# PreferredAI/cornac

Measured on AMD Instinct MI355X. Metric: bpr_triplets_per_sec, higher is better.
Workload: dtype f32

## Files before the change

cornac_amd/csrc/bpr.hip:

```cpp
#include <algorithm>
#include <numeric>
#include <queue>

#include "common.h"
#include "rng.h"
#include "sgd_device.h"

namespace chip {

__global__ __launch_bounds__(kBlock) void bpr_det_sample_kernel(
    const uint32_t *__restrict__ pos_draw, int pos_stride, const uint32_t *__restrict__ neg_draw, int neg_stride,
    int64_t n, const int32_t *__restrict__ user_ids, const int32_t *__restrict__ indices,
    const int32_t *__restrict__ indptr, int neg_population, int32_t *__restrict__ su, int32_t *__restrict__ si,
    int32_t *__restrict__ sj, unsigned long long *__restrict__ counters) {
    const int64_t s = (int64_t)blockIdx.x * kBlock + threadIdx.x;
    bool skip = false;
    if (s < n) {
        const uint32_t ii = pos_draw[s * pos_stride];
        const uint32_t jj = neg_draw[s * neg_stride];
        const int32_t u = user_ids[ii];
        const int32_t i = indices[ii];
        const int32_t j = neg_population == CORNAC_HIP_NEG_POPULARITY ? indices[jj] : (int32_t)jj;
        skip = csr_row_contains(indices, indptr[u], indptr[u + 1], j);
        su[s] = skip ? -1 : u;
// ... 1474 lines not shown
    const int grid = di.cus * h->strata_blocks_per_cu;
    const int64_t W = (int64_t)grid * kWavesPerBlock;
    if (h->own_waves != W) h->strata_built = false;
    build_ownership(h, W);
    build_item_ranks(h);
    h->rec_u.ensure((size_t)h->nnz);
    h->rec_i.ensure((size_t)h->nnz);
    h->sptr.ensure((size_t)W * 8 + 1);
    REQUIRE(grid % 8 == 0, "the strata grid must be a multiple of the 8 XCDs");
    h->strata_claim.ensure(8 * 16);
    return grid;
}

static void strata_build_buckets(cornac_hip_bpr_t h, int grid, uint32_t key) {
    if (h->strata_built && h->strata_key_built == key) return;
    StrataArgs s;
    s.own_u = h->own_u.p; s.own_i = h->own_i.p; s.wave_ptr = h->wave_ptr.p; s.item_rank = h->item_rank.p;
    s.rec_u = h->rec_u.p; s.rec_i = h->rec_i.p; s.sptr = h->sptr.p;
    s.key = key; s.n_hot = h->strata_n_hot; s.n_waves = (int64_t)grid * kWavesPerBlock;
    h->strata_own_code.ensure((size_t)h->nnz);
    s.own_code = h->strata_own_code.p;
    if (h->strata_code_waves != h->own_waves) {
        hipLaunchKernelGGL(strata_code_kernel, dim3((unsigned)std::min<int64_t>(4096, (h->nnz + kBlock - 1) / kBlock)),
                           dim3(kBlock), 0, h->stream, s, h->nnz);
        h->strata_code_waves = h->own_waves;
    }
    hipLaunchKernelGGL(strata_bucket_kernel, dim3(grid), dim3(kBlock), 0, h->stream, s);
    HIP_CHECK(hipGetLastError());
    h->strata_built = true;
    h->strata_key_built = key;
    ++h->strata_builds;
}

static void strata_enqueue(cornac_hip_bpr_t h, int64_t n_samples, float lr, float reg, int use_bias, int flags) {
    const int grid = strata_prepare(h);
    const bool packed = h->strata_allow_pack && ((h->V.owned && h->B.owned) || h->chunk_records) &&
                        !prof_env_set("CORNAC_HIP_STRATA_NO_PACK");
    if (packed) strata_pack(h); else strata_unpack(h);
    if (!packed) h->Bpad.ensure((size_t)h->total_items * kBiasStride);
    const unsigned bgrid = (unsigned)((h->total_items + kBlock - 1) / kBlock);
    int64_t left = n_samples;
    while (left > 0) {
        const int64_t n = std::min(left, h->nnz - h->hog_offset);
        const auto first_phase = [&](int64_t s) { return (int)((8 * (__int128)s + h->nnz - 1) / h->nnz); };
        const int p_lo = first_phase(h->hog_offset), p_hi = h->hog_offset + n >= h->nnz ? 8 : first_phase(h->hog_offset + n);
        if (p_hi > p_lo) {
            uint32_t key = strata_key(h->hog_seed, h->hog_epoch / (uint32_t)std::max(1, h->strata_rehash_period));
            if (prof_env_int("CORNAC_HIP_STRATA_CONTIG", 0)) key = 0x12345u;
            strata_build_buckets(h, grid, key);
            HogArgs a;
            fill_hog_args(h, a, h->nnz, lr, reg, use_bias, CORNAC_HIP_NEG_UNIFORM, flags);
            const bool dense_bias = !packed && prof_env_int("CORNAC_HIP_STRATA_DENSE_BIAS", 0) != 0;
            a.B = dense_bias ? h->B.p : h->Bpad.p;
            a.bstride = dense_bias ? 1 : kBiasStride;
            if (packed) {
                a.V = h->VB.p;
                a.vpitch = h->vb_pitch;
                a.B = h->VB.p + h->vb_kp;
                a.bstride = h->vb_pitch;
            }
            a.rec_u = h->rec_u.p; a.rec_i = h->rec_i.p; a.rank_item = h->rank_item.p; a.sptr = h->sptr.p;
            a.strata_key = key; a.n_hot = h->strata_n_hot;
            HIP_CHECK(hipMemsetAsync(h->strata_claim.p, 0, 8 * 16 * sizeof(uint32_t), h->stream));
            if (!dense_bias && !packed)
                hipLaunchKernelGGL(bias_pad_kernel, dim3(bgrid), dim3(kBlock), 0, h->stream, h->B.p, h->Bpad.p, h->total_items);
            for (int ph = p_lo; ph < p_hi; ++ph) {
                a.phase = ph;
                a.xcd_claim = h->strata_claim.p + 16 * ph;
                h->ktimer.before(h->stream);
                hipLaunchKernelGGL(h->strata_kernel, dim3(grid), dim3(kBlock), 0, h->stream, a);
                h->ktimer.after(h->stream);
            }
            if (!dense_bias && !packed)
                hipLaunchKernelGGL(bias_unpad_kernel, dim3(bgrid), dim3(kBlock), 0, h->stream, h->Bpad.p, h->B.p, h->total_items);
            HIP_CHECK(hipGetLastError());
        }
        advance_hog_offset(h, n);
        left -= n;
    }
}

typedef void (*LdsBinKernel)(const LdsBinArgs);
constexpr int kLdsbinPresampleDefault = 0;
static LdsBinKernel pick_ldsbin_kernel(int k, bool pop, bool exch = false, bool passing = false, bool conv = false, bool pre = false) {
    if (pre) {
        if (k <= 64) return bpr_ldsbin_kernel<1, 4, false, false, 1, false, true>;
        return bpr_ldsbin_kernel<2, 2, false, false, 1, false, true>;
    }
    if (conv) {
        if (pop) {
            if (k <= 64) return bpr_ldsbin_kernel<1, 4, true, false, 1, true>;
            if (k <= 128) return bpr_ldsbin_kernel<2, 4, true, false, 1, true>;
            if (k <= 192) return bpr_ldsbin_kernel<3, 2, true, false, 1, true>;
            return bpr_ldsbin_kernel<4, 1, true, false, 1, true>;
        }
        if (k <= 64) return bpr_ldsbin_kernel<1, 4, false, false, 1, true>;
        if (k <= 128) return bpr_ldsbin_kernel<2, 4, false, false, 1, true>;
        if (k <= 192) return bpr_ldsbin_kernel<3, 2, false, false, 1, true>;
        return bpr_ldsbin_kernel<4, 1, false, false, 1, true>;
    }
    if (passing && !exch && k > 64 && k <= 128) {
#ifdef CORNAC_PROFILE
        if (prof_env_int("CORNAC_HIP_LDSBIN_UNR", 0) == 0)
#endif
            return pop ? bpr_ldsbin_kernel<2, 4, true> : bpr_ldsbin_kernel<2, 4>;
    }
    if (exch) {
        if (pop) {
            if (k <= 64) return bpr_ldsbin_kernel<1, 4, true, true>;
            if (k <= 128) return bpr_ldsbin_kernel<2, 2, true, true>;
            if (k <= 192) return bpr_ldsbin_kernel<3, 2, true, true>;
            return bpr_ldsbin_kernel<4, 1, true, true>;
        }
        if (k <= 64) return bpr_ldsbin_kernel<1, 4, false, true>;
        if (k <= 128) return bpr_ldsbin_kernel<2, 2, false, true>;
        if (k <= 192) return bpr_ldsbin_kernel<3, 2, false, true>;
        return bpr_ldsbin_kernel<4, 1, false, true>;
    }
    if (pop) {
        if (k <= 64) return bpr_ldsbin_kernel<1, 4, true>;
        if (k <= 128) return bpr_ldsbin_kernel<2, 2, true>;
        if (k <= 192) return bpr_ldsbin_kernel<3, 2, true>;
        return bpr_ldsbin_kernel<4, 1, true>;
    }
#ifdef CORNAC_PROFILE
    if (k <= 64) switch (prof_env_int("CORNAC_HIP_LDSBIN_UNR", 0)) {
        case 1: return bpr_ldsbin_kernel<1, 1>;
        case 2: return bpr_ldsbin_kernel<1, 2>;
        case 8: return bpr_ldsbin_kernel<1, 8>;
        default: break;
    }
    else if (k <= 128) switch (prof_env_int("CORNAC_HIP_LDSBIN_UNR", 0)) {
        case 3: return bpr_ldsbin_kernel<2, 3>;
        case 4: return bpr_ldsbin_kernel<2, 4>;
        case 22: return bpr_ldsbin_kernel<2, 2, false, false, 2>;
        case 32: return bpr_ldsbin_kernel<2, 3, false, false, 2>;
        case 42: return bpr_ldsbin_kernel<2, 4, false, false, 2>;
        default: break;
    }
#endif
    if (k <= 64) return bpr_ldsbin_kernel<1, 4>;
    if (k <= 128) return bpr_ldsbin_kernel<2, 2>;
    if (k <= 192) return bpr_ldsbin_kernel<3, 2>;
    return bpr_ldsbin_kernel<4, 1>;
}

constexpr size_t kLbLdsBudget = 96 * 1024;
constexpr size_t kLbLdsExclusive = 82 * 1024;
static size_t ldsbin_lds_bytes(int cap, int k, int waves = kLbWaves) {
    const int kp = ((k + kWave - 1) / kWave) * kWave;
    return ((size_t)cap * (kp + 5) + 1) * sizeof(float) + (size_t)waves * 3 * kWave * sizeof(int32_t);
}

struct LbPlan {
    int bins = 0, block = kLbBlock, cap = 0;
    size_t lds = 0;
    bool passing = false;
};
static LbPlan ldsbin_plan(cornac_hip_bpr_t h) {
    LbPlan pl;
    const int cus = device_info(h->device).cus;
    if (h->cv_blocks) {
        if (h->k > 256) return pl;
        const int waves = h->lb_pass_waves;
        const size_t budget = (size_t)h->lb_pass_kb << 10;
        const int kp = ((h->k + kWave - 1) / kWave) * kWave;
        const size_t fixed = sizeof(float) + (size_t)waves * 3 * kWave * sizeof(int32_t);
        if (budget <= fixed) return pl;
        const int64_t cap_lds = (int64_t)((budget - fixed) / ((size_t)(kp + 5) * sizeof(float)));
        const int64_t cap_min = std::max<int64_t>(h->lb_min_candidates, 16);
        if (cap_lds < cap_min) return pl;
        int64_t bins = (h->n_items + cap_lds - 1) / cap_lds;
        const int64_t more = std::min<int64_t>(h->n_items / (cap_min + cap_min / 3), (int64_t)2 * cus * h->cv_blocks);
        bins = std::max(bins, more);
        bins = std::max<int64_t>(1, (bins + h->cv_blocks - 1) / h->cv_blocks) * h->cv_blocks;
        const int64_t cap = (h->n_items + bins - 1) / bins;
        if (cap > cap_lds || bins > (int64_t(1) << 22) || bins * cap >= (int64_t(1) << 31)) return pl;
        pl.bins = (int)bins;
        pl.cap = (int)cap;
        pl.block = waves * kWave;
        pl.lds = ldsbin_lds_bytes((int)cap, h->k, waves);
        pl.passing = true;
        return pl;
    }
    if (h->k > 256 || h->nnz < (int64_t)cus * kLbWaves * kWave) return pl;
    const int res_waves = prof_env_int("CORNAC_HIP_LDSBIN_RES_WAVES", kLbWaves);
    for (int rounds = prof_env_int("CORNAC_HIP_LDSBIN_MIN_ROUNDS", 1); rounds <= h->lb_max_rounds; ++rounds) {
        const int64_t bins = (int64_t)cus * rounds;
        const int64_t cap = (h->n_items + bins - 1) / bins;
        if (cap < h->lb_min_candidates) return pl;
        if (ldsbin_lds_bytes((int)cap, h->k, res_waves) <= (size_t)prof_env_int("CORNAC_HIP_LDSBIN_BUDGET_KB", (int)(kLbLdsBudget >> 10)) << 10) {
            pl.bins = (int)bins;
            pl.cap = (int)cap;
            pl.block = res_waves * kWave;
            pl.lds = std::max(ldsbin_lds_bytes((int)cap, h->k, res_waves), (size_t)prof_env_int("CORNAC_HIP_LDSBIN_EXCL_KB", (int)(kLbLdsExclusive >> 10)) << 10);
            return pl;
        }
    }
    if (!h->lb_pass_enable || (double)h->nnz * 100.0 < (double)h->n_items * h->lb_pass_min_draws_x100) return pl;
    const int waves = prof_env_int("CORNAC_HIP_LDSBIN_PASS_WAVES", h->lb_pass_waves);
    const size_t budget = (size_t)prof_env_int("CORNAC_HIP_LDSBIN_PASS_KB", h->lb_pass_kb) << 10;
    const int kp = ((h->k + kWave - 1) / kWave) * kWave;
    const size_t fixed = sizeof(float) + (size_t)waves * 3 * kWave * sizeof(int32_t);
    if (budget <= fixed) return pl;
    int64_t cap = (int64_t)((budget - fixed) / ((size_t)(kp + 5) * sizeof(float)));
    if (cap < h->lb_min_candidates) return pl;
    int64_t bins = (h->n_items + cap - 1) / cap;
    bins = ((bins + cus - 1) / cus) * cus;
    cap = (h->n_items + bins - 1) / bins;
    if (cap < h->lb_min_candidates || bins > (int64_t(1) << 22)) return pl;
    pl.bins = (int)bins;
    pl.cap = (int)cap;
    pl.block = waves * kWave;
    pl.lds = ldsbin_lds_bytes((int)cap, h->k, waves);
    pl.passing = true;
    return pl;
}

static bool ldsbin_can_run(cornac_hip_bpr_t h, int64_t n_samples, int neg_population) {
    if (neg_population == CORNAC_HIP_NEG_POPULARITY && h->neg_pop_n) return false;
    const LbPlan pl = ldsbin_plan(h);
    return pl.bins > 0 && (!pl.passing || n_samples * 4 >= h->nnz);
}

static void ldsbin_build(cornac_hip_bpr_t h) {
    const LbPlan plan = ldsbin_plan(h);
    const int bins = plan.bins;
// ... 768 lines not shown
```

cornac_amd/csrc/bpr_ldsbin.inc:

```


namespace chip {

constexpr int kLbBlock = 1024;
constexpr int kLbWaves = kLbBlock / kWave;
constexpr int32_t kLbHot = (int32_t)0x80000000;
constexpr int kLbMaxExchanges = 32;
constexpr int kLbMaxRanges = 8;

struct LdsBinExchange {
    float *base;
    float *bucket;
    float *keep;
    unsigned int *arrive;
    const unsigned int *landed;
    unsigned int *applied;
    long long bucket_stride, keep_stride;
    long long nt;
    int n_ex, rule;
};

struct LdsBinArgs {
    const int32_t *cptr, *cusers;
    const int32_t *rank_item;
    const int32_t *hot_u, *hot_i;
    const uint32_t *hot_off;
    const int32_t *indptr, *indices;
    const uint32_t *bitmap;
    float *U, *V, *B;
    unsigned long long *counters;
    uint64_t seed;
    uint32_t epoch, key;
    int32_t n_items, n_bins, n_hot, n_hot_inter, bm_words, cap;
    int32_t n_strata;
    unsigned long long *wg_clock;
    int k, use_bias;
    float lr, reg;
    int ablate;
    int neg_pop;
    uint64_t s_begin, n, nnz;
    LdsBinExchange ex;
    int32_t conv_bpb;
    int32_t conv_first[kLbMaxRanges];
    float *conv_rows[kLbMaxRanges];
    int32_t *pre_rec;
    uint32_t *pre_cnt;
    const uint32_t *pre_base;
    uint32_t pre_waves;
};

__host__ __device__ __forceinline__ uint32_t ldsbin_rot(uint32_t g, uint32_t key, uint32_t n_bins) {
    uint32_t h = g * 0x9E3779B1u + key;
    h ^= h >> 15; h *= 0x85EBCA77u;
    h ^= h >> 13; h *= 0xC2B2AE3Du;
    h ^= h >> 16;
    return h % n_bins;
}

__host__ __device__ __forceinline__ uint32_t ldsbin_mix(uint32_t h) { return mix32(h); }
__host__ __device__ __forceinline__ uint32_t ldsbin_perm(uint32_t x, uint32_t n, uint32_t key) { return feistel_perm(x, n, key); }

__host__ __device__ inline uint32_t ldsbin_deal_rank(uint32_t p, uint32_t key, uint32_t n_bins, uint32_t n_items,
                                                     uint32_t n_groups, uint32_t n_strata) {
    const uint32_t g = p / n_bins;
    uint32_t s = (uint32_t)(((uint64_t)g * n_strata) / n_groups);
    if ((uint32_t)(((uint64_t)(s + 1u) * n_groups) / n_strata) <= g) ++s;
    const uint32_t g_lo = (uint32_t)(((uint64_t)s * n_groups) / n_strata);
    const uint32_t g_hi = (uint32_t)(((uint64_t)(s + 1u) * n_groups) / n_strata);
    const uint32_t base = g_lo * n_bins;
    const uint64_t end = (uint64_t)g_hi * n_bins;
    const uint32_t size = (uint32_t)(end < (uint64_t)n_items ? end : (uint64_t)n_items) - base;
    return base + ldsbin_perm(p - base, size, key ^ ldsbin_mix(s * 0x27D4EB2Fu + 0x165667B1u));
}

#ifdef CORNAC_PROFILE
#define LB_ABLATE(bit) ((a.ablate & (bit)) != 0)
#else
#define LB_ABLATE(bit) false
#endif

__host__ __device__ __forceinline__ float ex_rule_factor(int rule, float w_sum, float s_norm2) {
    if (rule == 0) return 1.f / sqrtf(fmaxf(w_sum, 1.f));
    return s_norm2 > 0.f ? fminf(1.f, w_sum / s_norm2) : 1.f;
}
__device__ __forceinline__ void store_f32_system(float *p, float v) {
// ... 233 lines not shown
        uint32_t run = 0;
        for (uint32_t g0 = 0; g0 < n_groups; g0 += kWave) {
            const uint32_t g = g0 + lane;
            uint32_t v = g < n_groups ? cum[g + 1] : 0u;
#pragma unroll
            for (int o = 1; o < kWave; o <<= 1) {
                const uint32_t t = __shfl_up(v, o, kWave);
                if (lane >= o) v += t;
            }
            if (g < n_groups) cum[g + 1] = run + v;
            run += __shfl(v, kWave - 1, kWave);
        }
        if (lane == 0) {
            cum[0] = 0;
            *sh_next_tile = 0;
            *sh_cold_mass = run;
            *sh_nslots = (n_groups && item[n_groups - 1] == -1) ? n_groups - 1 : n_groups;
        }
    }
    __syncthreads();
}

template <bool POP>
__device__ __forceinline__ LdsBinDraw ldsbin_draw(const LdsBinArgs &a, const LdsBinCtx &c, uint32_t local, bool in_range) {
    LdsBinDraw d;
    d.in_range = in_range;
    uint32_t w[4];
    philox4x32_10(d.in_range ? local : 0u, c.b, a.epoch, 0x20u, (uint32_t)a.seed, (uint32_t)(a.seed >> 32), w);
    const uint32_t r_pos = lemire_bounded2(w[0], w[1], c.n_draws, c.th_draw);
    uint32_t s_j, excl = 0, excl_lo = 0xffffffffu;
    if (r_pos < c.cold_mass) {
        uint32_t lo = 0, hi = c.n_slots;
        while (hi - lo > 1) {
            const uint32_t mid = (lo + hi) >> 1;
            if (c.cum[mid] <= r_pos) lo = mid; else hi = mid;
        }
        d.u = a.cusers[c.cp[lo] + (int32_t)(r_pos - c.cum[lo])];
        d.ei = (int32_t)lo;
        s_j = c.n_slots > 1 ? lemire_bounded2(w[2], w[3], c.n_slots - 1, c.th_slot1) : 0u;
        if (c.n_slots > 1 && s_j >= lo) ++s_j;
        excl_lo = c.cum[lo];
        excl = c.cum[lo + 1] - excl_lo;
    } else {
        const uint32_t h = c.hot_lo + (r_pos - c.cold_mass);
        d.u = a.hot_u[h];
        d.ei = a.hot_i[h] | kLbHot;
        s_j = lemire_bounded2(w[2], w[3], c.n_slots, c.th_slot);
    }
    if (POP) {
        const uint32_t m = c.n_draws - excl;
        uint32_t r_neg = (uint32_t)(((uint64_t)w[2] * m) >> 32);
        if (r_neg >= excl_lo) r_neg += excl;
        if (m == 0) {
            d.j = c.item[d.ei] & ~kLbHot;
            d.ej = d.ei;
        } else if (r_neg < c.cold_mass) {
            uint32_t lo = 0, hi = c.n_slots;
            while (hi - lo > 1) {
                const uint32_t mid = (lo + hi) >> 1;
                if (c.cum[mid] <= r_neg) lo = mid; else hi = mid;
            }
            d.j = c.item[lo];
            d.ej = (int32_t)lo;
        } else {
            d.j = a.hot_i[c.hot_lo + (r_neg - c.cold_mass)];
            d.ej = d.j | kLbHot;
        }
        return d;
    }
    const int32_t itj = c.item[s_j];
    d.j = itj & ~kLbHot;
    d.ej = itj < 0 ? itj : (int32_t)s_j;
    return d;
}

__device__ __forceinline__ void ldsbin_launch_range(const LdsBinArgs &a, uint32_t n_draws, uint32_t n_waves, uint32_t &d_lo,
                                                    uint32_t &d_hi, uint32_t &tile_w, uint32_t &n_tiles) {
    d_lo = (uint32_t)(((unsigned __int128)n_draws * a.s_begin) / a.nnz);
    d_hi = a.s_begin + a.n >= a.nnz ? n_draws : (uint32_t)(((unsigned __int128)n_draws * (a.s_begin + a.n)) / a.nnz);
    tile_w = (d_hi - d_lo) < 8u * n_waves * kWave ? 32u : 64u;
    n_tiles = (d_hi - d_lo + tile_w - 1) / tile_w;
}

template <int R, int UNR, bool POP = false, bool EXCH = false, int PF = 1, bool CONV = false, bool PRE = false>
__global__ __launch_bounds__(kLbBlock) void bpr_ldsbin_kernel(const LdsBinArgs a) {
    constexpr int G = kWave, KP = G * R, NREF = 2 * UNR;
    extern __shared__ float lb_smem[];
    float *const rows = lb_smem;
    float *const bias = rows + (size_t)a.cap * KP;
    int32_t *const item = reinterpret_cast<int32_t *>(bias + a.cap);
    int32_t *const cp = item + a.cap;
    uint32_t *const cum = reinterpret_cast<uint32_t *>(cp + a.cap);
    int *const lock = reinterpret_cast<int *>(cum + a.cap + 1);
    int32_t(*const stage)[3][kWave] = reinterpret_cast<int32_t(*)[3][kWave]>(lock + a.cap);
    const int wave = threadIdx.x >> 6, lane = lane_id();
    const uint32_t n_waves = blockDim.x >> 6;
    uint32_t b = blockIdx.x;
    const uint32_t nb = (uint32_t)a.n_bins;
    float *cvV = nullptr, *cvB = nullptr;
    if (CONV) {
        const uint32_t r = blockIdx.x / (uint32_t)a.conv_bpb, o = blockIdx.x - r * (uint32_t)a.conv_bpb;
        b = (uint32_t)a.conv_first[r] + o;
        cvV = a.conv_rows[r] + (size_t)o * (size_t)a.cap * (size_t)a.k;
        cvB = a.conv_rows[r] + (size_t)a.conv_bpb * (size_t)a.cap * (size_t)a.k + (size_t)o * (size_t)a.cap;
    }
    const uint32_t n_groups = ((uint32_t)a.n_items + nb - 1) / nb;
#ifdef CORNAC_PROFILE
    if (a.wg_clock && threadIdx.x == 0) a.wg_clock[2 * b] = wall_clock64();
#endif
    __shared__ uint32_t sh_nslots, sh_cold_mass, sh_next_tile;
    __shared__ uint32_t sh_ex_done[kLbMaxExchanges], sh_ex_applied[kLbWaves];
    __shared__ int sh_ex_lock[kLbWaves];
    if (EXCH) {
        if (threadIdx.x < kLbMaxExchanges) sh_ex_done[threadIdx.x] = 0;
        if (threadIdx.x < kLbWaves) {
            sh_ex_applied[threadIdx.x] = 0;
            sh_ex_lock[threadIdx.x] = 0;
        }
    }
    ldsbin_build_tables(a, b, nb, n_groups, item, cp, cum, lock, &sh_nslots, &sh_cold_mass, &sh_next_tile);
    const uint32_t n_slots = sh_nslots, cold_mass = sh_cold_mass;
    const uint32_t hot_lo = a.hot_off[b], hot_share = a.hot_off[b + 1] - hot_lo;
    const uint32_t n_draws = n_slots ? cold_mass + hot_share : 0u;
    const uint32_t th_draw = n_draws ? lemire_thresh(n_draws) : 0u, th_slot = n_slots ? lemire_thresh(n_slots) : 0u,
                   th_slot1 = n_slots > 1 ? lemire_thresh(n_slots - 1) : 0u;
    bool inb[R];
#pragma unroll
    for (int r = 0; r < R; ++r) inb[r] = lane + G * r < a.k;
    {
        constexpr int NL = R <= 2 ? 4 : 2;
        for (uint32_t s0 = wave; s0 < n_slots; s0 += n_waves * NL) {
            float t[NL][R], tb[NL];
            int32_t its[NL];
#pragma unroll
            for (int q = 0; q < NL; ++q) {
                const uint32_t sq = s0 + (uint32_t)q * n_waves;
                its[q] = sq < n_slots ? item[sq] : -1;
                const size_t it = (size_t)(its[q] >= 0 ? its[q] : 0);
                const float *pv = CONV ? cvV + (size_t)(its[q] >= 0 ? sq : 0u) * a.k : a.V + it * a.k;
                const float *pb = CONV ? cvB + (its[q] >= 0 ? sq : 0u) : a.B + it;
#pragma unroll
                for (int r = 0; r < R; ++r) t[q][r] = (its[q] >= 0 && inb[r]) ? pv[lane + G * r] : 0.f;
                tb[q] = (its[q] >= 0 && lane == 0) ? *pb : 0.f;
            }
#pragma unroll
            for (int q = 0; q < NL; ++q) {
                if (its[q] < 0) continue;
                const uint32_t sq = s0 + (uint32_t)q * n_waves;
#pragma unroll
                for (int r = 0; r < R; ++r) rows[(size_t)sq * KP + lane + G * r] = t[q][r];
                if (lane == 0) bias[sq] = tb[q];
            }
        }
    }
    __syncthreads();
    unsigned int n_correct = 0, n_skipped = 0;
    if (!PRE && n_slots == 0 && wave == 0 && lane == 0 && a.s_begin == 0) n_skipped = cold_mass + hot_share;
    uint32_t d_lo, d_hi, tile_w, n_tiles;
    ldsbin_launch_range(a, n_draws, n_waves, d_lo, d_hi, tile_w, n_tiles);
    const LdsBinCtx ctx{item, cp, cum, b, n_slots, cold_mass, hot_lo, n_draws, th_draw, th_slot, th_slot1};
    typedef LdsBinDraw Draws;
    auto draw_tile = [&](uint32_t tile) {
        const uint32_t local = d_lo + tile * tile_w + lane;
        return ldsbin_draw<POP>(a, ctx, local, tile < n_tiles && (uint32_t)lane < tile_w && local < d_hi);
    };
    auto member_word = [&](const Draws &d) -> uint32_t {
        return (a.bitmap && !LB_ABLATE(1)) ? a.bitmap[(size_t)d.u * a.bm_words + (d.j >> 5)] : 0u;
    };
    auto member_bounds = [&](const Draws &d, int32_t &lo, int32_t &hi) {
        lo = hi = 0;
        if (!a.bitmap && !LB_ABLATE(1) && d.in_range) {
            lo = a.indptr[d.u];
            hi = a.indptr[d.u + 1];
        }
    };
    auto claim_tile = [&]() -> uint32_t {
        uint32_t t = 0;
        if (lane == 0) t = atomicAdd(&sh_next_tile, 1u);
        return (uint32_t)__builtin_amdgcn_readfirstlane((int)t);
    };
    const uint32_t ex_per = EXCH ? n_tiles / (uint32_t)a.ex.n_ex : 0u;
    const uint32_t ex_parts = ex_per < n_waves ? ex_per : n_waves;
    auto ex_landed_upto = [&](int from, int below) -> int {
        int e = from;
        if (lane == 0)
            while (e < below && __hip_atomic_load(a.ex.landed + e, __ATOMIC_RELAXED, __HIP_MEMORY_SCOPE_SYSTEM) != 0u) ++e;
        return __builtin_amdgcn_readfirstlane(e);
    };
    auto ex_duty = [&](uint32_t t) {
        if (!EXCH || ex_parts == 0u || t >= n_tiles) return;
        const uint32_t q = t / ex_per, part = t - q * ex_per;
        if (q == 0u || q >= (uint32_t)a.ex.n_ex || part >= ex_parts) return;
        const int e = (int)q - 1;
        if (lane == 0)
            while (atomicCAS(&sh_ex_lock[part], 0, 1) != 0) __builtin_amdgcn_s_sleep(2);
        __builtin_amdgcn_fence(__ATOMIC_ACQUIRE, "workgroup");
        const int e_lo = (int)sh_ex_applied[part];
        const int e_hi = ex_landed_upto(e_lo, e);
        if (e_hi > e_lo) __builtin_amdgcn_fence(__ATOMIC_ACQUIRE, "agent");
        constexpr int NB = R == 1 ? 4 : 2;
        if (!LB_ABLATE(64)) {
            for (uint32_t s = part; s < n_slots; s += ex_parts) {
                const int32_t it = item[s];
                if (it >= 0)
                    ex_row_duty<R>(a.ex, a.V, a.B, a.k, it, rows + (size_t)s * KP, bias + s, lock + s, e_lo, e_hi, e, lane, inb, a.counters + 3);
            }
        } else
        for (uint32_t s0 = part; s0 < n_slots; s0 += ex_parts * NB) {
            int32_t its[NB];
            float *lrow[NB], *lbias[NB];
            int *llock[NB];
#pragma unroll
            for (int q = 0; q < NB; ++q) {
                const uint32_t s = s0 + (uint32_t)q * ex_parts;
                const uint32_t sc = s < n_slots ? s : s0;
                const int32_t it = item[sc];
                its[q] = (s < n_slots && it >= 0) ? it : -1;
                lrow[q] = rows + (size_t)sc * KP;
                lbias[q] = bias + sc;
                llock[q] = lock + sc;
            }
            ex_rows_duty<R, NB>(a.ex, a.k, its, lrow, lbias, llock, e_lo, e_hi, e, lane, inb, a.counters + 3);
        }
        if (part == 0u)
            for (uint32_t hr = b; hr < (uint32_t)a.n_hot; hr += nb)
                ex_row_duty<R>(a.ex, a.V, a.B, a.k, a.rank_item[hr], nullptr, nullptr, nullptr, e_lo, e_hi, e, lane, inb, a.counters + 3);
        asm volatile("s_waitcnt vmcnt(0)" ::: "memory");
        if (lane == 0) {
            sh_ex_applied[part] = (uint32_t)e_hi;
            __builtin_amdgcn_fence(__ATOMIC_RELEASE, "workgroup");
            __hip_atomic_store(&sh_ex_lock[part], 0, __ATOMIC_RELAXED, __HIP_MEMORY_SCOPE_WORKGROUP);
            if (atomicAdd(&sh_ex_done[e], 1u) == ex_parts - 1u)
                __hip_atomic_fetch_add(a.ex.arrive + e, 1u, __ATOMIC_RELAXED, __HIP_MEMORY_SCOPE_SYSTEM);
        }
    };
    auto train_tile = [&](const int nvalid) __attribute__((always_inline)) {
        float u_nx[PF][UNR][R];
        int32_t tu_nx[PF][UNR];
        auto request_users = [&](float (&ub)[UNR][R], int32_t (&tub)[UNR], int t0) {
#pragma unroll
            for (int q = 0; q < UNR; ++q) {
                const int sl = t0 + q < nvalid ? t0 + q : (t0 < nvalid ? t0 : 0);
                tub[q] = __builtin_amdgcn_readfirstlane(stage[wave][0][sl]);
#pragma unroll
                for (int r = 0; r < R; ++r)
                    ub[q][r] = !inb[r] || LB_ABLATE(4) ? 0.f
                               : LB_ABLATE(8)          ? load_f32_fresh(a.U + (size_t)tub[q] * a.k + lane + G * r)
                                                       : __builtin_nontemporal_load(a.U + (size_t)tub[q] * a.k + lane + G * r);
            }
        };
        auto step = [&](float (&ub)[UNR][R], int32_t (&tub)[UNR], int t0) {
            float u_[UNR][R], v_[NREF][R], bv[NREF];
            float *pu[UNR];
            int32_t ref[NREF];
            bool act[UNR];
#pragma unroll
            for (int q = 0; q < UNR; ++q) {
                act[q] = t0 + q < nvalid;
                const int sl = act[q] ? t0 + q : t0;
                ref[2 * q] = __builtin_amdgcn_readfirstlane(stage[wave][1][sl]);
                ref[2 * q + 1] = __builtin_amdgcn_readfirstlane(stage[wave][2][sl]);
                pu[q] = a.U + (size_t)tub[q] * a.k + lane;
#pragma unroll
                for (int r = 0; r < R; ++r) u_[q][r] = ub[q][r];
            }
            if (t0 + PF * UNR < nvalid) request_users(ub, tub, t0 + PF * UNR);
#pragma unroll
            for (int c = 0; c < NREF; ++c) {
                if (ref[c] < 0) {
                    const int32_t it = ref[c] & ~kLbHot;
#pragma unroll
                    for (int r = 0; r < R; ++r) v_[c][r] = inb[r] ? load_f32_fresh(a.V + (size_t)it * a.k + lane + G * r) : 0.f;
                    bv[c] = load_f32_fresh(a.B + it);
                } else {
#pragma unroll
                    for (int r = 0; r < R; ++r) v_[c][r] = rows[(size_t)ref[c] * KP + lane + G * r];
                    bv[c] = bias[ref[c]];
                }
            }
            float du[UNR][R], zq[UNR];
#pragma unroll
            for (int q = 0; q < UNR; ++q) {
                float part = 0.f;
#pragma unroll
                for (int r = 0; r < R; ++r) part += u_[q][r] * (v_[2 * q][r] - v_[2 * q + 1][r]);
                const float score = (bv[2 * q] - bv[2 * q + 1]) + (LB_ABLATE(256) ? part : LB_ABLATE(1024) ? group_sum<G>(part) : wave_sum_dpp(part));
                const float z = LB_ABLATE(512) ? 0.5f + 1e-3f * score : sigmoid_neg_fast(score);
                zq[q] = z;
#pragma unroll
                for (int r = 0; r < R; ++r) du[q][r] = a.lr * (z * (v_[2 * q][r] - v_[2 * q + 1][r]) - a.reg * u_[q][r]);
                if (act[q] && lane == 0) n_correct += z < .5f ? 1u : 0u;
            }
#pragma unroll
            for (int q = 0; q < UNR; ++q) {
                if (!act[q] || LB_ABLATE(2)) continue;
#pragma unroll
                for (int r = 0; r < R; ++r)
                    if (inb[r]) {
                        if (LB_ABLATE(8)) store_f32_agent(pu[q] + G * r, u_[q][r] + du[q][r]);
                        else if (LB_ABLATE(16)) pu[q][G * r] = u_[q][r] + du[q][r];
                        else atomic_add_f32(pu[q] + G * r, du[q][r]);
                    }
            }
#pragma unroll
            for (int c = 0; c < NREF; ++c) {
                const int q = c >> 1;
                if (!act[q] || LB_ABLATE(2)) continue;
                const float zs = (c & 1) ? -zq[q] : zq[q];
                if (ref[c] < 0) {
                    const int32_t it = ref[c] & ~kLbHot;
#pragma unroll
                    for (int r = 0; r < R; ++r)
                        if (inb[r]) atomic_add_f32(a.V + (size_t)it * a.k + lane + G * r, a.lr * (zs * u_[q][r] - a.reg * v_[c][r]));
                    if (a.use_bias && lane == 0) atomic_add_f32(a.B + it, a.lr * (zs - a.reg * bv[c]));
                    continue;
                }
                const int s = ref[c];
                if (LB_ABLATE(32)) continue;
                if (!EXCH && LB_ABLATE(2048)) {
#pragma unroll
                    for (int r = 0; r < R; ++r)
                        atomicAdd(rows + (size_t)s * KP + lane + G * r, a.lr * (zs * u_[q][r] - a.reg * v_[c][r]));
                    if (a.use_bias && lane == 0) atomicAdd(bias + s, a.lr * (zs - a.reg * bv[c]));
                    continue;
                }
                const bool owned = LB_ABLATE(128) ? false : lds_row_lock(&lock[s], lane, a.counters + 3);
#pragma unroll
                for (int r = 0; r < R; ++r) {
                    float *pv = rows + (size_t)s * KP + lane + G * r;
                    const float v = *pv;
                    *pv = v + a.lr * (zs * u_[q][r] - a.reg * v);
                }
                if (a.use_bias && lane == 0) {
                    const float bb = bias[s];
                    bias[s] = bb + a.lr * (zs - a.reg * bb);
                }
                if (!LB_ABLATE(128)) lds_row_unlock(&lock[s], lane, owned);
            }
        };
        if (nvalid) request_users(u_nx[0], tu_nx[0], 0);
        if (PF == 2 && UNR < nvalid) request_users(u_nx[PF - 1], tu_nx[PF - 1], UNR);
        for (int t0 = 0; t0 < nvalid; t0 += PF * UNR) {
            step(u_nx[0], tu_nx[0], t0);
            if (PF == 2 && t0 + UNR < nvalid) step(u_nx[PF - 1], tu_nx[PF - 1], t0 + UNR);
        }
    };
    if constexpr (PRE) {
        const size_t pool0 = (size_t)a.pre_base[b];
        int32_t rec[3] = {0, 0, 0};
        uint32_t cnt = 0;
        auto fetch = [&](uint32_t t) {
            if (t < n_tiles) {
                const size_t o = pool0 + t;
                cnt = a.pre_cnt[o];
#pragma unroll
                for (int q = 0; q < 3; ++q) rec[q] = a.pre_rec[(o * 3 + q) * kWave + lane];
            }
        };
        uint32_t tB = n_tiles ? claim_tile() : 0u;
        fetch(tB);
        while (tB < n_tiles) {
            const int nvalid = __builtin_amdgcn_readfirstlane((int)cnt);
#pragma unroll
            for (int q = 0; q < 3; ++q) stage[wave][q][lane] = rec[q];
            __builtin_amdgcn_fence(__ATOMIC_ACQ_REL, "wavefront");
            __builtin_amdgcn_wave_barrier();
            tB = claim_tile();
            fetch(tB);
            train_tile(nvalid);
            __builtin_amdgcn_wave_barrier();
        }
    } else {
    uint32_t tB = n_tiles ? claim_tile() : 0u;
    Draws dB = n_tiles ? draw_tile(tB) : Draws{0, 0, 0, 0, false};
    if (n_tiles) ex_duty(tB);
    uint32_t tA = n_tiles ? claim_tile() : 0u;
    Draws dA = n_tiles ? draw_tile(tA) : dB;
    if (n_tiles) ex_duty(tA);
    uint32_t wordB = (n_tiles && dB.in_range) ? member_word(dB) : 0u;
    int32_t rowB_lo, rowB_hi;
    member_bounds(dB, rowB_lo, rowB_hi);
    while (tB < n_tiles) {
        bool skip = (wordB >> (dB.j & 31)) & 1u;
        if (!a.bitmap && !LB_ABLATE(1) && dB.in_range) skip = csr_row_contains(a.indices, rowB_lo, rowB_hi, dB.j);
        const bool valid = dB.in_range && !skip;
        const unsigned long long mask = __ballot(valid);
        n_skipped += (dB.in_range && !valid) ? 1u : 0u;
        if (valid) {
            const int pos = __popcll(mask & ((1ull << lane) - 1ull));
            stage[wave][0][pos] = dB.u;
            stage[wave][1][pos] = dB.ei;
            stage[wave][2][pos] = dB.ej;
        }
        __builtin_amdgcn_fence(__ATOMIC_ACQ_REL, "wavefront");
        __builtin_amdgcn_wave_barrier();
        const int nvalid = __popcll(mask);
        dB = dA;
        tB = tA;
        wordB = dB.in_range ? member_word(dB) : 0u;
        member_bounds(dB, rowB_lo, rowB_hi);
        tA = claim_tile();
        dA = draw_tile(tA);
        ex_duty(tA);
        train_tile(nvalid);
        __builtin_amdgcn_wave_barrier();
    }
    }
    __syncthreads();
    if (EXCH) {
        const int n_ex = a.ex.n_ex;
        const int landed_hi = ex_landed_upto(0, n_ex - 1);
        if (landed_hi > 0) __builtin_amdgcn_fence(__ATOMIC_ACQUIRE, "agent");
        for (int e = ex_parts ? n_ex - 1 : 0; e < n_ex; ++e) {
            const bool first = e == (ex_parts ? n_ex - 1 : 0);
            for (uint32_t s = wave; s < n_slots; s += n_waves) {
                const int32_t it = item[s];
                if (it < 0) continue;
                const int lo = ex_parts ? (int)sh_ex_applied[s % ex_parts] : 0;
                const int hi = ex_parts ? (landed_hi > lo ? landed_hi : lo) : 0;
                ex_row_duty<R>(a.ex, a.V, a.B, a.k, it, rows + (size_t)s * KP, bias + s, nullptr, first ? lo : hi, hi, e, lane, inb, a.counters + 3);
                if (lane == 0) a.ex.applied[it] = (unsigned int)hi;
            }
            if (wave == 0)
                for (uint32_t hr = b; hr < (uint32_t)a.n_hot; hr += nb) {
                    const int32_t it = a.rank_item[hr];
                    const int lo = ex_parts ? (int)sh_ex_applied[0] : 0;
                    const int hi = ex_parts ? (landed_hi > lo ? landed_hi : lo) : 0;
                    ex_row_duty<R>(a.ex, a.V, a.B, a.k, it, nullptr, nullptr, nullptr, first ? lo : hi, hi, e, lane, inb, a.counters + 3);
                    if (lane == 0) a.ex.applied[it] = (unsigned int)hi;
                }
            asm volatile("s_waitcnt vmcnt(0)" ::: "memory");
            __syncthreads();
            if (threadIdx.x == 0) __hip_atomic_fetch_add(a.ex.arrive + e, 1u, __ATOMIC_RELAXED, __HIP_MEMORY_SCOPE_SYSTEM);
        }
    }
    for (uint32_t s = wave; s < n_slots; s += n_waves) {
        const int32_t it = item[s];
        if (it >= 0) {
            float *pv = CONV ? cvV + (size_t)s * a.k : a.V + (size_t)it * a.k;
#pragma unroll
            for (int r = 0; r < R; ++r)
                if (inb[r]) pv[lane + G * r] = rows[(size_t)s * KP + lane + G * r];
            if (lane == 0) *(CONV ? cvB + s : a.B + it) = bias[s];
        }
    }
#pragma unroll
    for (int o = 32; o > 0; o >>= 1) {
        n_correct += __shfl_xor(n_correct, o, kWave);
        n_skipped += __shfl_xor(n_skipped, o, kWave);
    }
    if (lane == 0) {
        if (n_correct) atomicAdd(&a.counters[0], (unsigned long long)n_correct);
        if (n_skipped) atomicAdd(&a.counters[1], (unsigned long long)n_skipped);
    }
#ifdef CORNAC_PROFILE
    __syncthreads();
    if (a.wg_clock && threadIdx.x == 0) a.wg_clock[2 * b + 1] = wall_clock64();
#endif
}

struct LdsTileBaseArgs {
    const uint32_t *cold, *hot_off;
    uint32_t *base;
    uint64_t s_begin, n, nnz;
    int32_t n_bins;
    uint32_t n_waves;
};

__global__ __launch_bounds__(kLbBlock) void ldsbin_tilebase_kernel(const LdsTileBaseArgs t) {
    __shared__ uint32_t carry;
    if (threadIdx.x == 0) carry = 0;
    __syncthreads();
    const int wave = threadIdx.x >> 6, lane = lane_id();
    (void)wave;
    for (int32_t b0 = 0; b0 < t.n_bins; b0 += kLbBlock) {
        const int32_t b = b0 + (int32_t)threadIdx.x;
        uint32_t tiles = 0;
        if (b < t.n_bins) {
            const uint32_t n_draws = t.cold[b] + (t.hot_off[b + 1] - t.hot_off[b]);
            const uint32_t d_lo = (uint32_t)(((unsigned __int128)n_draws * t.s_begin) / t.nnz);
            const uint32_t d_hi = t.s_begin + t.n >= t.nnz ? n_draws : (uint32_t)(((unsigned __int128)n_draws * (t.s_begin + t.n)) / t.nnz);
            const uint32_t tile_w = (d_hi - d_lo) < 8u * t.n_waves * kWave ? 32u : 64u;
            tiles = (d_hi - d_lo + tile_w - 1) / tile_w;
        }
        __shared__ uint32_t wsum[kLbWaves];
        uint32_t v = tiles;
#pragma unroll
// ... 276 lines not shown
```

Baseline: 3.412 billion.

## Partition staged triplets into cold/hot groups and specialize full-k kernels

Staged triplets are partitioned within each wave so that triplets touching only LDS-resident (cold) items come first and those with hot items come last. Cold steps are compiled without the per-reference hot branch and the global-memory fallback, and a tail of single-triplet steps handles the remainder without masked padding. A FULL template variant is also added, selected when k equals the padded width, which drops the per-lane bounds predicate. This roughly doubles the instantiated kernel variants, raising code size and compile time, and adds extra ballots per tile.

New measurement: 3.353 billion. -1.7%, worse.

```diff
diff --git a/cornac_amd/csrc/bpr.hip b/cornac_amd/csrc/bpr.hip
--- a/cornac_amd/csrc/bpr.hip
+++ b/cornac_amd/csrc/bpr.hip
@@ -1580,67 +1580,74 @@
 
 typedef void (*LdsBinKernel)(const LdsBinArgs);
 constexpr int kLdsbinPresampleDefault = 0;
+template <int R, int UNR, bool POP = false, bool EXCH = false, int PF = 1, bool CONV = false, bool PRE = false>
+static LdsBinKernel ldsbin_inst(int k) {
+    if (k == kWave * R) return bpr_ldsbin_kernel<R, UNR, POP, EXCH, PF, CONV, PRE, true>;
+    return bpr_ldsbin_kernel<R, UNR, POP, EXCH, PF, CONV, PRE, false>;
+}
 static LdsBinKernel pick_ldsbin_kernel(int k, bool pop, bool exch = false, bool passing = false, bool conv = false, bool pre = false) {
     if (pre) {
-        if (k <= 64) return bpr_ldsbin_kernel<1, 4, false, false, 1, false, true>;
-        return bpr_ldsbin_kernel<2, 2, false, false, 1, false, true>;
+        if (k <= 64) return ldsbin_inst<1, 4, false, false, 1, false, true>(k);
+        return ldsbin_inst<2, 2, false, false, 1, false, true>(k);
     }
     if (conv) {
         if (pop) {
-            if (k <= 64) return bpr_ldsbin_kernel<1, 4, true, false, 1, true>;
-            if (k <= 128) return bpr_ldsbin_kernel<2, 4, true, false, 1, true>;
-            if (k <= 192) return bpr_ldsbin_kernel<3, 2, true, false, 1, true>;
-            return bpr_ldsbin_kernel<4, 1, true, false, 1, true>;
-        }
-        if (k <= 64) return bpr_ldsbin_kernel<1, 4, false, false, 1, true>;
-        if (k <= 128) return bpr_ldsbin_kernel<2, 4, false, false, 1, true>;
-        if (k <= 192) return bpr_ldsbin_kernel<3, 2, false, false, 1, true>;
-        return bpr_ldsbin_kernel<4, 1, false, false, 1, true>;
+            if (k <= 64) return ldsbin_inst<1, 4, true, false, 1, true>(k);
+            if (k <= 128) return ldsbin_inst<2, 4, true, false, 1, true>(k);
+            if (k <= 192) return ldsbin_inst<3, 2, true, false, 1, true>(k);
+            return ldsbin_inst<4, 1, true, false, 1, true>(k);
+        }
+        if (k <= 64) return ldsbin_inst<1, 4, false, false, 1, true>(k);
+        if (k <= 128) return ldsbin_inst<2, 4, false, false, 1, true>(k);
+        if (k <= 192) return ldsbin_inst<3, 2, false, false, 1, true>(k);
+        return ldsbin_inst<4, 1, false, false, 1, true>(k);
     }
     if (passing && !exch && k > 64 && k <= 128) {
 #ifdef CORNAC_PROFILE
         if (prof_env_int("CORNAC_HIP_LDSBIN_UNR", 0) == 0)
 #endif
-            return pop ? bpr_ldsbin_kernel<2, 4, true> : bpr_ldsbin_kernel<2, 4>;
+            return pop ? ldsbin_inst<2, 4, true>(k) : ldsbin_inst<2, 4>(k);
     }
     if (exch) {
         if (pop) {
-            if (k <= 64) return bpr_ldsbin_kernel<1, 4, true, true>;
-            if (k <= 128) return bpr_ldsbin_kernel<2, 2, true, true>;
-            if (k <= 192) return bpr_ldsbin_kernel<3, 2, true, true>;
-            return bpr_ldsbin_kernel<4, 1, true, true>;
-        }
-        if (k <= 64) return bpr_ldsbin_kernel<1, 4, false, true>;
-        if (k <= 128) return bpr_ldsbin_kernel<2, 2, false, true>;
-        if (k <= 192) return bpr_ldsbin_kernel<3, 2, false, true>;
-        return bpr_ldsbin_kernel<4, 1, false, true>;
+            if (k <= 64) return ldsbin_inst<1, 4, true, true>(k);
+            if (k <= 128) return ldsbin_inst<2, 2, true, true>(k);
+            if (k <= 192) return ldsbin_inst<3, 2, true, true>(k);
+            return ldsbin_inst<4, 1, true, true>(k);
+        }
+        if (k <= 64) return ldsbin_inst<1, 4, false, true>(k);
+        if (k <= 128) return ldsbin_inst<2, 2, false, true>(k);
+        if (k <= 192) return ldsbin_inst<3, 2, false, true>(k);
+        return ldsbin_inst<4, 1, false, true>(k);
     }
     if (pop) {
-        if (k <= 64) return bpr_ldsbin_kernel<1, 4, true>;
-        if (k <= 128) return bpr_ldsbin_kernel<2, 2, true>;
-        if (k <= 192) return bpr_ldsbin_kernel<3, 2, true>;
-        return bpr_ldsbin_kernel<4, 1, true>;
+        if (k <= 64) return ldsbin_inst<1, 4, true>(k);
+        if (k <= 128) return ldsbin_inst<2, 2, true>(k);
+        if (k <= 192) return ldsbin_inst<3, 2, true>(k);
+        return ldsbin_inst<4, 1, true>(k);
     }
 #ifdef CORNAC_PROFILE
     if (k <= 64) switch (prof_env_int("CORNAC_HIP_LDSBIN_UNR", 0)) {
-        case 1: return bpr_ldsbin_kernel<1, 1>;
-        case 2: return bpr_ldsbin_kernel<1, 2>;
-        case 8: return bpr_ldsbin_kernel<1, 8>;
+        case 1: return ldsbin_inst<1, 1>(k);
+        case 2: return ldsbin_inst<1, 2>(k);
+        case 8: return ldsbin_inst<1, 8>(k);
+        case 22: return ldsbin_inst<1, 2, false, false, 2>(k);
+        case 42: return ldsbin_inst<1, 4, false, false, 2>(k);
         default: break;
     }
     else if (k <= 128) switch (prof_env_int("CORNAC_HIP_LDSBIN_UNR", 0)) {
-        case 3: return bpr_ldsbin_kernel<2, 3>;
-        case 4: return bpr_ldsbin_kernel<2, 4>;
-        case 22: return bpr_ldsbin_kernel<2, 2, false, false, 2>;
-        case 32: return bpr_ldsbin_kernel<2, 3, false, false, 2>;
-        case 42: return bpr_ldsbin_kernel<2, 4, false, false, 2>;
+        case 3: return ldsbin_inst<2, 3>(k);
+        case 4: return ldsbin_inst<2, 4>(k);
+        case 22: return ldsbin_inst<2, 2, false, false, 2>(k);
+        case 32: return ldsbin_inst<2, 3, false, false, 2>(k);
+        case 42: return ldsbin_inst<2, 4, false, false, 2>(k);
         default: break;
     }
 #endif
-    if (k <= 64) return bpr_ldsbin_kernel<1, 4>;
-    if (k <= 128) return bpr_ldsbin_kernel<2, 2>;
-    if (k <= 192) return bpr_ldsbin_kernel<3, 2>;
-    return bpr_ldsbin_kernel<4, 1>;
+    if (k <= 64) return ldsbin_inst<1, 4>(k);
+    if (k <= 128) return ldsbin_inst<2, 2>(k);
+    if (k <= 192) return ldsbin_inst<3, 2>(k);
+    return ldsbin_inst<4, 1>(k);
 }
 
 constexpr size_t kLbLdsBudget = 96 * 1024;
diff --git a/cornac_amd/csrc/bpr_ldsbin.inc b/cornac_amd/csrc/bpr_ldsbin.inc
--- a/cornac_amd/csrc/bpr_ldsbin.inc
+++ b/cornac_amd/csrc/bpr_ldsbin.inc
@@ -1,6 +1,14 @@
 
+
+#include <type_traits>
+#include <utility>
 
 namespace chip {
+
+template <int... I, class F>
+__device__ __forceinline__ void static_for(std::integer_sequence<int, I...>, F &&f) {
+    (f(std::integral_constant<int, I>{}), ...);
+}
 
 constexpr int kLbBlock = 1024;
 constexpr int kLbWaves = kLbBlock / kWave;
@@ -400,9 +408,9 @@
     n_tiles = (d_hi - d_lo + tile_w - 1) / tile_w;
 }
 
-template <int R, int UNR, bool POP = false, bool EXCH = false, int PF = 1, bool CONV = false, bool PRE = false>
+template <int R, int UNR, bool POP = false, bool EXCH = false, int PF = 1, bool CONV = false, bool PRE = false, bool FULL = false>
 __global__ __launch_bounds__(kLbBlock) void bpr_ldsbin_kernel(const LdsBinArgs a) {
-    constexpr int G = kWave, KP = G * R, NREF = 2 * UNR;
+    constexpr int G = kWave, KP = G * R;
     extern __shared__ float lb_smem[];
     float *const rows = lb_smem;
     float *const bias = rows + (size_t)a.cap * KP;
@@ -444,7 +452,7 @@
                    th_slot1 = n_slots > 1 ? lemire_thresh(n_slots - 1) : 0u;
     bool inb[R];
 #pragma unroll
-    for (int r = 0; r < R; ++r) inb[r] = lane + G * r < a.k;
+    for (int r = 0; r < R; ++r) inb[r] = FULL || lane + G * r < a.k;
     {
         constexpr int NL = R <= 2 ? 4 : 2;
         for (uint32_t s0 = wave; s0 < n_slots; s0 += n_waves * NL) {
@@ -552,13 +560,12 @@
                 __hip_atomic_fetch_add(a.ex.arrive + e, 1u, __ATOMIC_RELAXED, __HIP_MEMORY_SCOPE_SYSTEM);
         }
     };
-    auto train_tile = [&](const int nvalid) __attribute__((always_inline)) {
-        float u_nx[PF][UNR][R];
-        int32_t tu_nx[PF][UNR];
-        auto request_users = [&](float (&ub)[UNR][R], int32_t (&tub)[UNR], int t0) {
+    auto train_tile = [&](const int n_cold, const int nvalid) __attribute__((always_inline)) {
+        if (nvalid == 0) return;
+        auto request_users = [&](float (&ub)[UNR][R], int32_t (&tub)[UNR], int t0) __attribute__((always_inline)) {
 #pragma unroll
             for (int q = 0; q < UNR; ++q) {
-                const int sl = t0 + q < nvalid ? t0 + q : (t0 < nvalid ? t0 : 0);
+                const int sl = t0 + q < nvalid ? t0 + q : nvalid - 1;
                 tub[q] = __builtin_amdgcn_readfirstlane(stage[wave][0][sl]);
 #pragma unroll
                 for (int r = 0; r < R; ++r)
@@ -567,25 +574,29 @@
                                                        : __builtin_nontemporal_load(a.U + (size_t)tub[q] * a.k + lane + G * r);
             }
         };
-        auto step = [&](float (&ub)[UNR][R], int32_t (&tub)[UNR], int t0) {
-            float u_[UNR][R], v_[NREF][R], bv[NREF];
-            float *pu[UNR];
+        auto step = [&](auto n_c, auto cold_c, auto q0_c, float (&ub)[UNR][R], int32_t (&tub)[UNR], int t0, int t_end,
+                        auto prefetch) __attribute__((always_inline)) {
+            constexpr int N = decltype(n_c)::value, NREF = 2 * N, Q0 = decltype(q0_c)::value;
+            constexpr bool COLD = decltype(cold_c)::value;
+            static_assert(Q0 + N <= UNR, "the step's user rows lie in one register set");
+            float u_[N][R], v_[NREF][R], bv[NREF];
+            float *pu[N];
             int32_t ref[NREF];
-            bool act[UNR];
-#pragma unroll
-            for (int q = 0; q < UNR; ++q) {
-                act[q] = t0 + q < nvalid;
+            bool act[N];
+#pragma unroll
+            for (int q = 0; q < N; ++q) {
+                act[q] = COLD || t0 + q < t_end;
                 const int sl = act[q] ? t0 + q : t0;
                 ref[2 * q] = __builtin_amdgcn_readfirstlane(stage[wave][1][sl]);
                 ref[2 * q + 1] = __builtin_amdgcn_readfirstlane(stage[wave][2][sl]);
-                pu[q] = a.U + (size_t)tub[q] * a.k + lane;
-#pragma unroll
-                for (int r = 0; r < R; ++r) u_[q][r] = ub[q][r];
-            }
-            if (t0 + PF * UNR < nvalid) request_users(ub, tub, t0 + PF * UNR);
+                pu[q] = a.U + (size_t)tub[Q0 + q] * a.k + lane;
+#pragma unroll
+                for (int r = 0; r < R; ++r) u_[q][r] = ub[Q0 + q][r];
+            }
+            prefetch();
 #pragma unroll
             for (int c = 0; c < NREF; ++c) {
-                if (ref[c] < 0) {
+                if (!COLD && ref[c] < 0) {
                     const int32_t it = ref[c] & ~kLbHot;
 #pragma unroll
                     for (int r = 0; r < R; ++r) v_[c][r] = inb[r] ? load_f32_fresh(a.V + (size_t)it * a.k + lane + G * r) : 0.f;
@@ -596,9 +607,9 @@
                     bv[c] = bias[ref[c]];
                 }
             }
-            float du[UNR][R], zq[UNR];
-#pragma unroll
-            for (int q = 0; q < UNR; ++q) {
+            float du[N][R], zq[N];
+#pragma unroll
+            for (int q = 0; q < N; ++q) {
                 float part = 0.f;
 #pragma unroll
                 for (int r = 0; r < R; ++r) part += u_[q][r] * (v_[2 * q][r] - v_[2 * q + 1][r]);
@@ -610,7 +621,7 @@
                 if (act[q] && lane == 0) n_correct += z < .5f ? 1u : 0u;
             }
 #pragma unroll
-            for (int q = 0; q < UNR; ++q) {
+            for (int q = 0; q < N; ++q) {
                 if (!act[q] || LB_ABLATE(2)) continue;
 #pragma unroll
                 for (int r = 0; r < R; ++r)
@@ -625,7 +636,7 @@
                 const int q = c >> 1;
                 if (!act[q] || LB_ABLATE(2)) continue;
                 const float zs = (c & 1) ? -zq[q] : zq[q];
-                if (ref[c] < 0) {
+                if (!COLD && ref[c] < 0) {
                     const int32_t it = ref[c] & ~kLbHot;
 #pragma unroll
                     for (int r = 0; r < R; ++r)
@@ -656,12 +667,81 @@
                 if (!LB_ABLATE(128)) lds_row_unlock(&lock[s], lane, owned);
             }
         };
-        if (nvalid) request_users(u_nx[0], tu_nx[0], 0);
-        if (PF == 2 && UNR < nvalid) request_users(u_nx[PF - 1], tu_nx[PF - 1], UNR);
-        for (int t0 = 0; t0 < nvalid; t0 += PF * UNR) {
-            step(u_nx[0], tu_nx[0], t0);
-            if (PF == 2 && t0 + UNR < nvalid) step(u_nx[PF - 1], tu_nx[PF - 1], t0 + UNR);
-        }
+        constexpr std::integral_constant<int, UNR> unr_c{};
+        constexpr std::integral_constant<int, 1> one_c{};
+        constexpr std::integral_constant<int, 0> zero_c{};
+        constexpr std::true_type cold_c{};
+        constexpr std::false_type general_c{};
+        float u_nx[PF][UNR][R];
+        int32_t tu_nx[PF][UNR];
+        const int n_full = n_cold - n_cold % UNR;
+        auto cold_step = [&](float (&ub)[UNR][R], int32_t (&tub)[UNR], int t0) __attribute__((always_inline)) {
+            step(unr_c, cold_c, zero_c, ub, tub, t0, n_cold, [&]() __attribute__((always_inline)) { request_users(ub, tub, t0 + PF * UNR); });
+        };
+        request_users(u_nx[0], tu_nx[0], 0);
+        if (PF == 2) request_users(u_nx[PF - 1], tu_nx[PF - 1], UNR);
+        bool odd = false;
+        if constexpr (PF == 1) {
+            if (n_full) {
+                cold_step(u_nx[0], tu_nx[0], 0);
+                for (int t0 = UNR; t0 < n_full; t0 += UNR) cold_step(u_nx[0], tu_nx[0], t0);
+            }
+        } else {
+            int t0 = 0;
+            if (n_full >= 2 * UNR) {
+                cold_step(u_nx[0], tu_nx[0], 0);
+                cold_step(u_nx[1], tu_nx[1], UNR);
+                for (t0 = 2 * UNR; t0 + 2 * UNR <= n_full; t0 += 2 * UNR) {
+                    cold_step(u_nx[0], tu_nx[0], t0);
+                    cold_step(u_nx[1], tu_nx[1], t0 + UNR);
+                }
+            }
+            if (t0 < n_full) {
+                cold_step(u_nx[0], tu_nx[0], t0);
+                odd = true;
+            }
+        }
+        float u_r[UNR][R];
+        int32_t tu_r[UNR];
+#pragma unroll
+        for (int q = 0; q < UNR; ++q) {
+            tu_r[q] = odd ? tu_nx[PF - 1][q] : tu_nx[0][q];
+#pragma unroll
+            for (int r = 0; r < R; ++r) u_r[q][r] = odd ? u_nx[PF - 1][q][r] : u_nx[0][q][r];
+        }
+        float u_h[PF][UNR][R];
+        int32_t tu_h[PF][UNR];
+        request_users(u_h[0], tu_h[0], n_cold);
+        if (PF == 2 && n_cold + UNR < nvalid) request_users(u_h[PF - 1], tu_h[PF - 1], n_cold + UNR);
+        static_for(std::make_integer_sequence<int, UNR - 1>{}, [&](auto i_c) __attribute__((always_inline)) {
+            if (n_full + decltype(i_c)::value < n_cold)
+                step(one_c, cold_c, i_c, u_r, tu_r, n_full + decltype(i_c)::value, n_cold, []() {});
+        });
+        auto hot_step = [&](float (&ub)[UNR][R], int32_t (&tub)[UNR], int t0) __attribute__((always_inline)) {
+            step(unr_c, general_c, zero_c, ub, tub, t0, nvalid, [&]() __attribute__((always_inline)) {
+                if (t0 + PF * UNR < nvalid) request_users(ub, tub, t0 + PF * UNR);
+            });
+        };
+        for (int t0 = n_cold; t0 < nvalid; t0 += PF * UNR) {
+            hot_step(u_h[0], tu_h[0], t0);
+            if (PF == 2 && t0 + UNR < nvalid) hot_step(u_h[PF - 1], tu_h[PF - 1], t0 + UNR);
+        }
+    };
+    auto stage_partition = [&](bool valid, int32_t u, int32_t ei, int32_t ej, int &n_cold) -> int {
+        const bool hot = (ei | ej) < 0;
+        const unsigned long long m_cold = __ballot(valid && !hot), m_hot = __ballot(valid && hot);
+        const unsigned long long below = (1ull << lane) - 1ull;
+        n_cold = __popcll(m_cold);
+        const int nvalid = n_cold + __popcll(m_hot);
+        if (valid) {
+            const int pos = hot ? nvalid - 1 - __popcll(m_hot & below) : __popcll(m_cold & below);
+            stage[wave][0][pos] = u;
+            stage[wave][1][pos] = ei;
+            stage[wave][2][pos] = ej;
+        }
+        __builtin_amdgcn_fence(__ATOMIC_ACQ_REL, "wavefront");
+        __builtin_amdgcn_wave_barrier();
+        return nvalid;
     };
     if constexpr (PRE) {
         const size_t pool0 = (size_t)a.pre_base[b];
@@ -678,14 +758,11 @@
         uint32_t tB = n_tiles ? claim_tile() : 0u;
         fetch(tB);
         while (tB < n_tiles) {
-            const int nvalid = __builtin_amdgcn_readfirstlane((int)cnt);
-#pragma unroll
-            for (int q = 0; q < 3; ++q) stage[wave][q][lane] = rec[q];
-            __builtin_amdgcn_fence(__ATOMIC_ACQ_REL, "wavefront");
-            __builtin_amdgcn_wave_barrier();
+            int n_cold;
+            const int nvalid = stage_partition(lane < __builtin_amdgcn_readfirstlane((int)cnt), rec[0], rec[1], rec[2], n_cold);
             tB = claim_tile();
             fetch(tB);
-            train_tile(nvalid);
+            train_tile(n_cold, nvalid);
             __builtin_amdgcn_wave_barrier();
         }
     } else {
@@ -702,17 +779,9 @@
         bool skip = (wordB >> (dB.j & 31)) & 1u;
         if (!a.bitmap && !LB_ABLATE(1) && dB.in_range) skip = csr_row_contains(a.indices, rowB_lo, rowB_hi, dB.j);
         const bool valid = dB.in_range && !skip;
-        const unsigned long long mask = __ballot(valid);
         n_skipped += (dB.in_range && !valid) ? 1u : 0u;
-        if (valid) {
-            const int pos = __popcll(mask & ((1ull << lane) - 1ull));
-            stage[wave][0][pos] = dB.u;
-            stage[wave][1][pos] = dB.ei;
-            stage[wave][2][pos] = dB.ej;
-        }
-        __builtin_amdgcn_fence(__ATOMIC_ACQ_REL, "wavefront");
-        __builtin_amdgcn_wave_barrier();
-        const int nvalid = __popcll(mask);
+        int n_cold;
+        const int nvalid = stage_partition(valid, dB.u, dB.ei, dB.ej, n_cold);
         dB = dA;
         tB = tA;
         wordB = dB.in_range ? member_word(dB) : 0u;
@@ -720,7 +789,7 @@
         tA = claim_tile();
         dA = draw_tile(tA);
         ex_duty(tA);
-        train_tile(nvalid);
+        train_tile(n_cold, nvalid);
         __builtin_amdgcn_wave_barrier();
     }
     }
```
